# dyustc/CTC-Attention-Mispronunciation

Hardware: AMD Instinct MI355X
Metric: phoneme-frames/sec joint CTC-attn decode, 41-phone vocab (higher is better)
Workload: dtype f32 -- reference width (operands with all 24 significand bits, fp32 accumulate; see `accuracy`: closer to a float64 evaluation than ATen's own fp32): the large time-batched contractions (conv0/conv1, BiLSTM and text input projections) run on the bf16 matrix cores as f32x6 = each fp32 operand as thre

## Files before the change

ctc-attention-mispronunciation_amd/csrc/api.hip:

```cpp
#include <stdarg.h>
#include <stdio.h>
#include <string.h>

#include <functional>
#include <mutex>

#include "model.h"

namespace mdd {

static thread_local char g_err[512] = "";

void set_error(const char *fmt, ...) {
    va_list ap;
    va_start(ap, fmt);
    vsnprintf(g_err, sizeof(g_err), fmt, ap);
    va_end(ap);
}

struct DeviceGate {
    std::mutex mu;
    hipEvent_t done = nullptr;
    hipStream_t stream = nullptr;
    bool armed = false;
// ... 4 lines not shown
    SplitPtr s; s.hi = reinterpret_cast<unsigned short *>(b.p); s.lo = s.hi ? s.hi + n : nullptr; return s;
}
static const SplitPtr kNoSplit = {nullptr, nullptr};
static unsigned short *as_u16(const DeviceBuf &b) { return reinterpret_cast<unsigned short *>(b.p); }

static std::mutex g_prep_mu;

static int ensure(DeviceBuf &b, size_t n, hipStream_t zero_stream, bool *moved) {
    if (b.cap >= n) return MDD_OK;
    *moved = true;
    if (int rc = b.need(n)) return rc;
    b.cap = 0;
    MDD_HIP_CHECK(hipMemsetAsync(b.p, 0, n * sizeof(float), zero_stream));
    MDD_HIP_CHECK(hipStreamSynchronize(zero_stream));
    b.cap = n;
    return MDD_OK;
}

static ForwardPlan plan_of(const mdd_model *m, int B) { return plan_forward(m->cfg, m->precision, m->sw, m->fit, B); }

static int run_lstm(mdd_model *m, const LstmWeights &lw, LstmStepArgs a, hipStream_t st) {
    const ForwardPlan &p = m->plan;
    a.gx = m->gx.p; a.whh = lw.whh; a.hbuf = m->hbuf.p; a.cbuf = m->cbuf.p;
    a.H = m->cfg.hidden; a.packed = packed_whh(m->cfg);
    a.whh_split = lw.whh_s; a.hsplit = p.lstm == Lstm::StepX3 ? as_u16(m->hsplit) : nullptr;
    if (!p.gated) return launch_lstm_layer(a, st);
    unsigned short *hx = as_u16(m->hx);
    long long *stamps = m->sw.lstm_dbg && a.T > 100 ? reinterpret_cast<long long *>(m->hx.p + p.stamps_at) : nullptr;
    if (p.lstm == Lstm::X6) return launch_lstm_layer_x6(a, lw.whh_3, hx, m->sync_words.p, m->err_flag.p, st, stamps, m->sw.x6_redo_mask);
    if (p.lstm == Lstm::Granule) return launch_lstm_layer_granule(a, hx, m->sync_words.p, m->err_flag.p, st, stamps, m->sw.lstm_early);
    return launch_lstm_layer_f32(a, hx, m->sync_words.p, m->err_flag.p, st, stamps);
}

static LstmStepArgs lstm_raw_out(int T, int B, const int *seqlen, float *out, SplitPtr split) {
    LstmStepArgs a;
    a.T = T; a.B = B; a.seqlen = seqlen; a.out = out; a.out_raw = out; a.out_split = split;
    return a;
}
static LstmStepArgs lstm_folded_out(mdd_model *m, int n, int T, int B, const int *seqlen) {
    const ForwardPlan &p = m->plan;
    const bool x3 = p.precision == 1;
    const size_t n_out = (size_t)T * B * 2 * m->cfg.hidden;
    LstmStepArgs a;
    a.T = T; a.B = B; a.seqlen = seqlen;
    a.out = x3 || p.planes_out ? nullptr : m->act[n & 1].p; a.out_raw = m->taps ? m->tap_rnn[n].p : nullptr;
    if (p.planes_out) {
        a.out_planes = as_u16(m->p3); a.out_planes_stride = n_out;
    }
    a.out_split = x3 ? split_view(m->act_s[n & 1], n_out) : kNoSplit;
    a.oscale = m->weights->rnn[n + 1].scale; a.oshift = m->weights->rnn[n + 1].shift;
    return a;
}

struct ProjIn { const float *f32; SplitPtr split; bool planes_written; };
static int project(mdd_model *m, const ProjIn &in, int rows, int K, const LstmWeights &lw, const float *bias, hipStream_t st) {
    const int G2 = 8 * m->cfg.hidden;
    if (m->plan.proj == Gemm::Bf16x3) return launch_gemm_bf16x3(in.split, lw.wih_s, bias, m->gx.p, nullptr, rows, G2, K, K, K, G2, 1, 0, 0, 0, st);
    if (m->plan.proj == Gemm::F32x6) {
        if (!in.planes_written)
            if (int rc = launch_split3(in.f32, rows, K, K, as_u16(m->p3), st)) return rc;
        return launch_gemm_f32x6(as_u16(m->p3), (size_t)rows * K, lw.wih_3, (size_t)G2 * K, bias, m->gx.p, rows, G2, K, G2, st);
    }
    return launch_gemm_nt(in.f32, lw.wih, bias, m->gx.p, rows, G2, K, K, K, G2, 1, 0, 0, 0, st);
}

struct Stage { std::string name; int launches; double flops; std::function<int(hipStream_t)> run; };

static std::vector<Stage> forward_stages(mdd_model *m, const ForwardCall &call) {
    const mdd_config &c = m->cfg;
    const DecodeWeights *w = m->weights.get();
    const ForwardPlan p = m->plan;
    const float *x = call.x;
    const int B = call.B, T = call.T, L = call.L, Traw = call.Traw, Tp = T / 2, Lp = L;
    const int H = c.hidden, H2 = 2 * H, ch = c.channels, E = c.emb_dim, K0 = m->rnn_in(), nl = c.layers;
    const bool x3 = p.precision == 1, fused = p.conv != Conv::Separate;
    const size_t rows = (size_t)Tp * B, trows = (size_t)L * B;
    const auto split = [x3](const DeviceBuf &b, size_t n) { return x3 ? split_view(b, n) : kNoSplit; };
    const double step_flops = 2.0 * 2 * (double)B * H * 4 * H;
    std::vector<Stage> s;

    if (fused) {
        s.push_back({"conv_fused", 1, 2.0 * 9 * ch * (double)B * Tp * m->W2() * (ch + 6.0), [=](hipStream_t st) {
            if (p.conv == Conv::FusedX3)
                return launch_conv_fused(x, w->w_conv0, w->sc0, w->sh0, w->w_conv1_s, w->sc1, w->sh1, split_view(m->seq0_s, rows * K0), nullptr, B, T, Traw, st);
            return launch_conv_fused3(x, w->w_conv0, w->sc0, w->sh0, w->w_conv1_3, w->sc1, w->sh1, as_u16(m->p3), m->taps ? m->seq0.p : nullptr, B, T, Traw, st,
                                      p.conv == Conv::FusedX6Rowwise);
        }});
        s.push_back({"conv1_in_fused", 0, 0.0, [](hipStream_t) { return (int)MDD_OK; }});
    } else {
        s.push_back({"conv0", 1, 2.0 * 9 * ch * (double)B * T * m->W1(), [=](hipStream_t st) {
            return launch_conv0(x, w->w_conv0, w->sc0, w->sh0, m->y0.p, B, T, c.feat, ch, st);
        }});
        s.push_back({"conv1", 1, 2.0 * 9 * ch * ch * (double)B * Tp * m->W2(), [=](hipStream_t st) {
            return launch_conv1(m->y0.p, w->w_conv1t, w->sc1, w->sh1, x3 ? nullptr : m->seq0.p, split(m->seq0_s, rows * K0), B, T, m->W1(), ch, st);
        }});
    }

    for (int n = 0; n < nl; n++) {
        const LstmWeights *lw = &w->rnn[n];
        const int K = n == 0 ? K0 : H2;
        const ProjIn in = n == 0 ? ProjIn{m->seq0.p, split(m->seq0_s, rows * K), fused}
                                 : ProjIn{m->act[(n - 1) & 1].p, split(m->act_s[(n - 1) & 1], rows * K), p.planes_out};
        s.push_back({"gemm_ih" + std::to_string(n), 1, 2.0 * (double)Tp * B * 8 * H * K, [=](hipStream_t st) {
            return project(m, in, Tp * B, K, *lw, nullptr, st);
        }});
        const LstmStepArgs a = n == nl - 1 ? lstm_raw_out(Tp, B, call.tlen, m->xraw.p, split(m->x_s, rows * H2)) : lstm_folded_out(m, n, Tp, B, call.tlen);
        s.push_back({"lstm" + std::to_string(n), p.gated ? 1 : Tp, step_flops * Tp, [=](hipStream_t st) { return run_lstm(m, *lw, a, st); }});
    }

    const LstmWeights *tw = &w->rnn[nl];
    s.push_back({"embed", 1, 0.0, [=](hipStream_t st) {
        return launch_embed(w->emb, c.emb_rows, E, call.x1, B, L, x3 ? nullptr : m->embo.p, split(m->embo_s, trows * E), m->err_flag.p, st);
    }});
    s.push_back({"gemm_text", 1, 2.0 * (double)L * B * 8 * H * E, [=](hipStream_t st) {
        return project(m, ProjIn{m->embo.p, split(m->embo_s, trows * E), false}, L * B, E, *tw, w->t_bias, st);
    }});
    const LstmStepArgs ta = lstm_raw_out(L, B, call.llen, m->text.p, split(m->text_s, trows * H2));
    s.push_back({"lstm_text", p.gated ? 1 : L, step_flops * L, [=](hipStream_t st) { return run_lstm(m, *tw, ta, st); }});
    s.push_back({"gemm_key", 1, 2.0 * (double)L * B * H2 * H2, [=](hipStream_t st) {
        if (x3) {
            const SplitPtr ks = split_view(m->key_s, trows * H2);
            return launch_gemm_bf16x3(split_view(m->text_s, trows * H2), w->w_score_s, nullptr, nullptr, &ks, L * B, H2, H2, H2, H2, H2, 1, 0, 0, 0, st);
        }
        return launch_gemm_nt(m->text.p, w->w_score, nullptr, m->key.p, L * B, H2, H2, H2, H2, H2, 1, 0, 0, 0, st);
    }});
    s.push_back({"gemm_score", 1, 2.0 * (double)B * Tp * L * H2, [=](hipStream_t st) {
        if (x3) return launch_gemm_bf16x3(split_view(m->x_s, rows * H2), split_view(m->key_s, trows * H2), nullptr, m->S.p, nullptr, Tp, L, H2, B * H2, B * H2, Lp,
                                          B, H2, H2, (long)Tp * Lp, st);
        return launch_gemm_nt(m->xraw.p, m->key.p, nullptr, m->S.p, Tp, L, H2, B * H2, B * H2, Lp, B, H2, H2, (long)Tp * Lp, st);
    }});
    s.push_back({"attn_tail", 1, 2.0 * (double)B * Tp * ((double)L * H2 + 2.0 * H2 * c.num_class), [=](hipStream_t st) {
        return launch_attn_tail(m->S.p, Lp, m->xraw.p, m->text.p, w->fscale, w->fshift, w->w_fc, w->w_fcp, call.logp, Tp, B, L, H2, c.num_class, st, call.llen);
    }});
    return s;
}

int device_gate_enter(int device, hipStream_t st, bool *held) {
    *held = false;
    hipStreamCaptureStatus cs = hipStreamCaptureStatusNone;
    if (st && hipStreamIsCapturing(st, &cs) == hipSuccess && cs != hipStreamCaptureStatusNone) return MDD_OK;
    DeviceGate &g = g_gate[device & 63];
    g.mu.lock();
    *held = true;
    if (g.armed && g.stream != st) {
        hipError_t e = hipStreamWaitEvent(st, g.done, 0);
        if (e != hipSuccess) { g.mu.unlock(); *held = false; set_error("device gate: %s", hipGetErrorString(e)); return MDD_ERR_HIP; }
    }
    return MDD_OK;
}
int device_gate_leave(int device, hipStream_t st, bool held, int rc) {
    if (!held) return rc;
    DeviceGate &g = g_gate[device & 63];
    hipError_t e = hipSuccess;
    if (!g.done) e = hipEventCreateWithFlags(&g.done, hipEventDisableTiming);
    if (e == hipSuccess) e = hipEventRecord(g.done, st);
    if (e == hipSuccess) { g.armed = true; g.stream = st; }
    g.mu.unlock();
    if (e != hipSuccess && rc == MDD_OK) { set_error("device gate: %s", hipGetErrorString(e)); return MDD_ERR_HIP; }
    return rc;
}

}

using namespace mdd;

extern "C" const char *mdd_last_error(void) { return g_err; }
extern "C" int mdd_version(void) { return 100; }

extern "C" int mdd_create(const mdd_config *cfg, int device, mdd_model **out) {
// ... 292 lines not shown
```

ctc-attention-mispronunciation_amd/csrc/decode.hip:

```cpp
#include "mdd_internal.h"

namespace mdd {

__global__ __launch_bounds__(256) void greedy_kernel(const float *__restrict__ logp, int T, int B, int C,
                                                     const int32_t *__restrict__ len, int blank,
                                                     int32_t *__restrict__ ids, int32_t *__restrict__ nids) {
    extern __shared__ int am[];
    const int b = blockIdx.x, lane = threadIdx.x & 63, wave = threadIdx.x >> 6;
    int n = len[b];
    n = n < 0 ? 0 : (n > T ? T : n);
    for (int t = wave; t < n; t += 4) {
        const float *row = logp + ((size_t)t * B + b) * C;
        float bv = -INFINITY;
        int bi = 0x7fffffff;
        for (int c = lane; c < C; c += 64) {
            float v = row[c];
            if (v > bv || bi == 0x7fffffff) { bv = v; bi = c; }
        }
        for (int o = 32; o > 0; o >>= 1) {
            float ov = __shfl_xor(bv, o);
            int oi = __shfl_xor(bi, o);
            if (oi != 0x7fffffff && (bi == 0x7fffffff || ov > bv || (ov == bv && oi < bi))) { bv = ov; bi = oi; }
        }
        if (lane == 0) am[t] = bi;
    }
    __syncthreads();
    if (wave != 0) return;
    int count = 0;
    for (int base = 0; base < n; base += 64) {
        const int t = base + lane;
        bool keep = false;
        int a = 0;
        if (t < n) {
            a = am[t];
            keep = (a != blank) && !(t != 0 && a == am[t - 1]);
        }
        const unsigned long long mask = __ballot(keep);
        if (keep) ids[(size_t)b * T + count + __popcll(mask & ((1ull << lane) - 1ull))] = a;
        count += __popcll(mask);
    }
    if (lane == 0) nids[b] = count;
}

#define LOG_ZERO (-99999999.0)

__device__ __forceinline__ double log_add_prob(double lx, double ly) {
    const bool swap = (ly - lx) > 0.0;
    const double hi = swap ? ly : lx, lo = swap ? lx : ly;
    const double sum = hi + log(1 + exp(lo - hi));
    return lx <= LOG_ZERO ? ly : (ly <= LOG_ZERO ? lx : sum);
}

struct BeamMeta {
    double prTotal, prNonBlank, prBlank;
    unsigned long long hash, phash;
    int len, last;
};

constexpr int MAXBEAM = 64;

__device__ __forceinline__ void wave_argmax(double &v, int &ord) {
    for (int o = 32; o > 0; o >>= 1) {
        const double ov = __shfl_xor(v, o);
        const int oo = __shfl_xor(ord, o);
        if (ov > v || (ov == v && oo < ord)) { v = ov; ord = oo; }
    }
}

__global__ __launch_bounds__(256) void beam_prep_kernel(const float *__restrict__ logp, int T, int B, int C, int blank,
                                                        double *__restrict__ lp, unsigned char *__restrict__ flags) {
    const size_t n = (size_t)T * B * C;
    for (size_t i = (size_t)blockIdx.x * blockDim.x + threadIdx.x; i < n; i += (size_t)gridDim.x * blockDim.x) {
        const float p = (float)exp((double)logp[i]);
        lp[i] = p > 0.0f ? log((double)p) : -INFINITY;
        const size_t tb = i / C;
        if ((int)(i - tb * C) == blank) {
            unsigned char f = ((1.0f - p) < 0.1f) ? 0 : 1;
            const size_t t = tb / B;
            if (t > 0) {
                const float pprev = (float)exp((double)logp[i - (size_t)B * C]);
                if (pprev < 0.9f) f |= 2;
            }
// ... 518 lines not shown
            if (rank < keep) { sel_v[rank] = v; sel_x[rank] = cl_x[e]; }
        }
        BEAM_WAVE_SYNC();
        FSTAMP(8);
        if (DBG) ph[11] += nl;
        const int nxt = cur ^ 1;
        int r_new, app_k, app_at;
        {
            const int idx = sel_x[li];
            const double v = sel_v[li];
            i32x4 M4[FB / 4];
#pragma unroll
            for (int a = 0; a < FB / 4; a++) M4[a] = reinterpret_cast<const i32x4 *>(mslot)[a];
            const int r = min((int)(((float)idx + 0.5f) * invC), FB - 1), k = idx - r * C;
            const double cNBr = cNB[r], cBr = cB[r];
            const int len_r = m_len[cur][r], last_r = m_last[cur][r];
            const unsigned long long hash_r = m_hash[cur][r], phash_r = m_phash[cur][r];
            int fa = -1;
#pragma unroll
            for (int a = 0; a < FB; a++) fa = M4[a >> 2][a & 3] == idx ? a : fa;
            const double cNBa = cNB[max(fa, 0)], cBa = cB[max(fa, 0)];
            const bool isb = k == blank;
            r_new = r; app_k = isb ? -1 : k; app_at = len_r;
            if (lane < FB) {
                const bool on = lane < keep;
                m_T[nxt][lane] = v;
                m_NB[nxt][lane] = isb ? cNBr : (fa >= 0 ? cNBa : v);
                m_B[nxt][lane] = isb ? cBr : (fa >= 0 ? cBa : LOG_ZERO);
                m_len[nxt][lane] = on ? (isb ? len_r : len_r + 1) : -2;
                m_last[nxt][lane] = on ? (isb ? last_r : k) : -1;
                m_hash[nxt][lane] = isb ? hash_r : hash_r * 0x9E3779B97F4A7C15ull + (unsigned long long)(k + 1);
                m_phash[nxt][lane] = isb ? phash_r : hash_r;
            }
        }
        FSTAMP(9);
        {
            int rr[FB];
#pragma unroll
            for (int i = 0; i < FB; i++) rr[i] = __builtin_amdgcn_readlane(r_new, i);
            unsigned int *dstw = reinterpret_cast<unsigned int *>(pnext);
            for (int j = lane; j < nw; j += 64) {
                unsigned int w[FB];
#pragma unroll
                for (int i = 0; i < FB; i++) w[i] = srcw[rr[i] * nw + j];
#pragma unroll
                for (int i = 0; i < FB; i++) dstw[i * nw + j] = w[i];
            }
            BEAM_WAVE_SYNC();
            if (lane < keep && app_k >= 0) pnext[(size_t)lane * Tcap + app_at] = (unsigned char)app_k;
        }
        BEAM_WAVE_SYNC();
        cur = nxt;
        nb = keep;
        t = tn;
        FSTAMP(10);
    }
    BEAM_WAVE_SYNC();
    if (lane == 0) {
        int best = -1;
        double bestv = 0.0;
        for (int r = 0; r < nb && !err; r++) {
            const int ylen = m_len[cur][r];
            if (ylen == 0) { err = MDD_BEAM_INDEX_ERROR; break; }
            const double v = lmt[m_last[cur][r] * C1 + C];
            if (v != v) { err = MDD_BEAM_KEY_ERROR; break; }
            double pr = log_add_prob(LOG_ZERO, m_T[cur][r] + v * alpha);
            pr = pr * (1.0 / (double)(ylen ? ylen : 1));
            if (best < 0 || pr > bestv) { best = r; bestv = pr; }
        }
        status[b] = err;
        int n = 0;
        if (!err && best >= 0) {
            n = m_len[cur][best];
            const unsigned char *src = pref + (size_t)cur * FB * Tcap + (size_t)best * Tcap;
            for (int j = 0; j < n; j++) ids[(size_t)b * T + j] = src[j];
        }
        nids[b] = n;
        if (score) score[b] = err ? __builtin_nan("") : bestv;
        if (DBG) for (int i = 0; i < 12; i++) dbg[b * 12 + i] = ph[i];
    }
#undef FSTAMP
}

}

extern "C" int mdd_greedy(const float *logp_dev, int32_t T, int32_t B, int32_t C, const int32_t *len_dev, int32_t blank,
                          int32_t *ids_dev, int32_t *nids_dev, void *stream) {
    using namespace mdd;
    if (!logp_dev || !len_dev || !ids_dev || !nids_dev || T <= 0 || B <= 0 || C <= 0 || blank < 0 || blank >= C) {
        set_error("mdd_greedy: bad argument"); return MDD_ERR_ARG;
    }
    if ((size_t)T * 4 > 150 * 1024) { set_error("mdd_greedy: T=%d too long", T); return MDD_ERR_ARG; }
    hipLaunchKernelGGL(greedy_kernel, dim3(B), dim3(256), (size_t)T * sizeof(int), (hipStream_t)stream, logp_dev, T, B, C,
                       len_dev, blank, ids_dev, nids_dev);
    MDD_LAUNCH_CHECK();
    return MDD_OK;
}

extern "C" int mdd_beam(const float *logp_dev, int32_t T, int32_t B, int32_t C, const int32_t *len_dev, int32_t beam,
                        int32_t blank, const double *lm_dev, double lm_alpha, int32_t *ids_dev, int32_t *nids_dev,
                        int32_t *status_dev, double *score_dev, void *stream) {
    using namespace mdd;
    if (!logp_dev || !len_dev || !lm_dev || !ids_dev || !nids_dev || !status_dev || T <= 0 || B <= 0 || C <= 1 ||
        C > 256 || beam < 1 || beam > MAXBEAM || blank < 0 || blank >= C) {
        set_error("mdd_beam: bad argument (need 1<=beam<=64, 2<=C<=256)"); return MDD_ERR_ARG;
    }
    hipStream_t st = (hipStream_t)stream;
    const int Tcap = (T + 1 + 3) & ~3;
    const size_t lm_bytes = sizeof(double) * (size_t)(C + 1) * (C + 1);
    const size_t base = (sizeof(double) * 2 + sizeof(int)) * (size_t)beam * C + (size_t)(2 * beam + 1) * Tcap;
    const int lm_in_lds = (base + lm_bytes <= 96 * 1024) ? 1 : 0;
    const size_t smem = base + (lm_in_lds ? lm_bytes : 0);
    if (smem > 140 * 1024) { set_error("mdd_beam: beam*C / T too large for LDS (%zu B)", smem); return MDD_ERR_ARG; }
    static bool attr_set = false;
    if (!attr_set) {
        MDD_HIP_CHECK(hipFuncSetAttribute((const void *)beam_kernel, hipFuncAttributeMaxDynamicSharedMemorySize, 140 * 1024));
        attr_set = true;
    }
    double *lpw = nullptr;
    unsigned char *flags = nullptr;
    const size_t n = (size_t)T * B * C;
    MDD_HIP_CHECK(hipMallocAsync((void **)&lpw, n * sizeof(double) + (size_t)T * B, st));
    flags = reinterpret_cast<unsigned char *>(lpw + n);
    int grid = (int)((n + 255) / 256);
    if (grid > 2048) grid = 2048;
    hipLaunchKernelGGL(beam_prep_kernel, dim3(grid), dim3(256), 0, st, logp_dev, T, B, C, blank, lpw, flags);
    const int nslots = beam * C;
    if (beam <= FB && C <= 64 && nslots <= 1024 && !getenv("MDD_BEAM_GENERIC")) {
        const int NS = nslots <= 512 ? 8 : 16;
        const size_t lmb = beam_fast_lm_bytes(C);
        const size_t pw = (beam_fast_wave_bytes(NS, beam, Tcap) + 15) & ~(size_t)15;
        const size_t lds_max = 160 * 1024;
        static bool fattr = false;
        if (!fattr) {
            MDD_HIP_CHECK(hipFuncSetAttribute((const void *)beam_fast_kernel<8, false>, hipFuncAttributeMaxDynamicSharedMemorySize, (int)lds_max));
            MDD_HIP_CHECK(hipFuncSetAttribute((const void *)beam_fast_kernel<16, false>, hipFuncAttributeMaxDynamicSharedMemorySize, (int)lds_max));
            MDD_HIP_CHECK(hipFuncSetAttribute((const void *)beam_fast_kernel<8, true>, hipFuncAttributeMaxDynamicSharedMemorySize, (int)lds_max));
            MDD_HIP_CHECK(hipFuncSetAttribute((const void *)beam_fast_kernel<16, true>, hipFuncAttributeMaxDynamicSharedMemorySize, (int)lds_max));
            fattr = true;
        }
        if (lmb + pw > lds_max) { (void)hipFreeAsync(lpw, st); set_error("mdd_beam: T too long for LDS (%zu B)", lmb + pw); return MDD_ERR_ARG; }
        int W = (int)((lds_max - lmb) / pw);
        W = W > 4 ? 4 : W;
        if (B <= 64) W = 1;
        if (const char *we = getenv("MDD_BEAM_W")) { const int w = atoi(we); if (w >= 1 && w <= W) W = w; }
        const size_t fs = lmb + (size_t)W * pw;
        const dim3 grid_f((B + W - 1) / W), block_f(64 * W);
        long long *fdbg = getenv("MDD_BEAM_DBG") ? reinterpret_cast<long long *>(score_dev) + B : nullptr;
#define MDD_BEAM_FAST(NS_, DBG_) hipLaunchKernelGGL((beam_fast_kernel<NS_, DBG_>), grid_f, block_f, fs, st, lpw, flags, T, B, C, len_dev, beam, blank, \
                                                  lm_dev, lm_alpha, ids_dev, nids_dev, status_dev, score_dev, Tcap, fdbg)
        if (NS == 8) { if (fdbg) MDD_BEAM_FAST(8, true); else MDD_BEAM_FAST(8, false); }
        else { if (fdbg) MDD_BEAM_FAST(16, true); else MDD_BEAM_FAST(16, false); }
#undef MDD_BEAM_FAST
    } else
    hipLaunchKernelGGL(beam_kernel, dim3(B), dim3(64), smem, st, lpw, flags, T, B, C, len_dev, beam, blank, lm_dev, lm_alpha,
                       ids_dev, nids_dev, status_dev, score_dev, Tcap, lm_in_lds, getenv("MDD_BEAM_SKIP") ? atoi(getenv("MDD_BEAM_SKIP")) : 0,
                       getenv("MDD_BEAM_DBG") ? reinterpret_cast<long long *>(score_dev) + B : nullptr);
    hipError_t le = hipGetLastError();
    (void)hipFreeAsync(lpw, st);
    if (le != hipSuccess) { set_error("beam kernel launch failed: %s", hipGetErrorString(le)); return MDD_ERR_HIP; }
    return MDD_OK;
}
```

ctc-attention-mispronunciation_amd/csrc/frontend.hip:

```cpp
#include "mdd_internal.h"

namespace mdd {

__global__ void stack_skip_kernel(const float *__restrict__ raw, int T_raw, int D, int right, int skip, int kept,
                                  int T_out, float *__restrict__ out) {
    const int W = (right + 1) * D;
    const int b = blockIdx.y, i = blockIdx.x;
    const float *src = raw + (size_t)b * T_raw * D;
    float *dst = out + ((size_t)b * T_out + i) * W;
    for (int j = threadIdx.x; j < W; j += blockDim.x) {
        float v = 0.f;
        if (i < kept) {
            int r = j / D, c = j - r * D;
            int s = i * skip + r;
            if (s > T_raw - 1) s = T_raw - 1;
            v = src[(size_t)s * D + c];
        }
        dst[j] = v;
    }
}

int launch_stack_skip(const float *raw, int B, int T_raw, int D, int right, int skip, int n_down, float *out,
                      hipStream_t st) {
    if (B <= 0 || T_raw <= 0 || D <= 0 || right < 0) { set_error("stack_skip: bad shape"); return MDD_ERR_ARG; }
// ... 510 lines not shown
        if (tp + R < tp_end) load_x(tp + R, xnext);
        CM_T(3);
        __syncthreads();
        CM_T(4);
        f32x16 acc;
#pragma unroll
        for (int r = 0; r < 16; r++) acc[r] = 0.f;
        const int m = min(mt * 32 + li, W2 - 1);
        int slot[3];
#pragma unroll
        for (int kh = 0; kh < 3; kh++) { const int r = 2 * jr + kh + rot; slot[kh] = (r >= NY ? r - NY : r) * CF_NCOL * 64; }
        float *rt = red + (jr * 2 + mt) * 16 * 64;
        auto conv1 = [&](auto kc) {
            constexpr int KH2 = decltype(kc)::value;
#pragma unroll
            for (int i = 0; i < 9; i++) {
                const int kb = KH2 * 9 + i, kk = kb >> 1, kh = kk / 3, kw = kk - kh * 3;
                const int off = slot[kh] + cm_yoff(0, 2 * m + kw, (kb & 1) * 2 + half);
                const bf16x8 ah = *reinterpret_cast<const bf16x8 *>(yh + off);
                const bf16x8 am = *reinterpret_cast<const bf16x8 *>(ym + off);
                const bf16x8 al = *reinterpret_cast<const bf16x8 *>(yl + off);
                acc = __builtin_amdgcn_mfma_f32_32x32x16_bf16(am, bwm[i], acc, 0, 0, 0);
                acc = __builtin_amdgcn_mfma_f32_32x32x16_bf16(ah, bwl[i], acc, 0, 0, 0);
                acc = __builtin_amdgcn_mfma_f32_32x32x16_bf16(al, bwh[i], acc, 0, 0, 0);
                acc = __builtin_amdgcn_mfma_f32_32x32x16_bf16(ah, bwm[i], acc, 0, 0, 0);
                acc = __builtin_amdgcn_mfma_f32_32x32x16_bf16(am, bwh[i], acc, 0, 0, 0);
                acc = __builtin_amdgcn_mfma_f32_32x32x16_bf16(ah, bwh[i], acc, 0, 0, 0);
            }
#pragma unroll
            for (int r = 0; r < 8; r++) rt[((1 - KH2) * 8 + r) * 64 + lane] = acc[(1 - KH2) * 8 + r];
        };
        auto finish = [&](auto kc) {
            constexpr int KH2 = decltype(kc)::value;
            unsigned short *oh = ost + jr * 3 * ROW + li * W2 + mt * 32 + 4 * half, *om = oh + ROW, *ol = om + ROW;
            const bool cut = mt == 1 && half == 1;
#pragma unroll
            for (int r = KH2 * 8; r < KH2 * 8 + 8; r += 2) {
                float v[2];
#pragma unroll
                for (int e = 0; e < 2; e++) {
                    const float p = rt[(r + e) * 64 + lane];
                    v[e] = (KH2 == 0 ? acc[r + e] + p : p + acc[r + e]) * s1 + h1;
                    v[e] = v[e] > 0.f ? v[e] : 0.f;
                }
                unsigned hw, mw, lw;
                split3_pair(v[0], v[1], hw, mw, lw);
                const int wo = (r & 3) + 8 * (r >> 2);
                if (r < 13 || !cut) { oh[wo] = (unsigned short)hw; om[wo] = (unsigned short)mw; ol[wo] = (unsigned short)lw; }
                if (r + 1 < 13 || !cut) { oh[wo + 1] = (unsigned short)(hw >> 16); om[wo + 1] = (unsigned short)(mw >> 16); ol[wo + 1] = (unsigned short)(lw >> 16); }
            }
        };
        if (kh2 == 0) conv1(std::integral_constant<int, 0>{}); else conv1(std::integral_constant<int, 1>{});
        CM_T(5);
        __syncthreads();
        CM_T(6);
        if (tp + jr < tp_end) {
            if (kh2 == 0) finish(std::integral_constant<int, 0>{}); else finish(std::integral_constant<int, 1>{});
        }
        CM_T(7);
        __syncthreads();
        CM_T(8);
        const int nr = min(R, tp_end - tp);
        unsigned short *orow = out3 + (size_t)tp * B * 32;
#pragma unroll
        for (int k = 0; k < SPT; k++) {
            const int i = tid + 512 * k;
            if (i < nr * 3 * 244) *reinterpret_cast<u32x4 *>(orow + sdst[k]) = *reinterpret_cast<const u32x4 *>(ost + i * 8);
        }
        if (out_f32)
            for (int i = tid; i < nr * ROW; i += 512) {
                const int jj = i / ROW, c = i - jj * ROW;
                const unsigned short *oh = ost + jj * 3 * ROW;
                out_f32[((size_t)(tp + jj) * B + b) * ROW + c] =
                    (__uint_as_float((unsigned)oh[c] << 16) + __uint_as_float((unsigned)oh[ROW + c] << 16)) + __uint_as_float((unsigned)oh[2 * ROW + c] << 16);
            }
        CM_T(9);
    }
    if (STAMP && stamps && lane == 0 && blockIdx.x < 512)
        for (int i = 0; i < CM_NPH; i++) stamps[((size_t)blockIdx.x * 8 + wave) * CM_NPH + i] = sacc[i];
#undef CM_T
}

int launch_conv_fused(const float *x, const float *w0, const float *sc0, const float *sh0, SplitPtr w1, const float *sc1,
                      const float *sh1, SplitPtr out, float *out_f32, int B, int T, int Traw, hipStream_t st) {
    const int Tp = T / 2;
    if (Tp <= 0 || B <= 0) return MDD_OK;
    int S = (1024 + B - 1) / B;
    S = S < 1 ? 1 : (S > Tp ? Tp : S);
    const int seg = (Tp + S - 1) / S;
    S = (Tp + seg - 1) / seg;
    hipLaunchKernelGGL(conv_fused_kernel<2>, dim3(B * S), dim3(256), conv_fused_smem(2), st, x, w0, sc0, sh0, w1.hi, w1.lo, sc1, sh1,
                       out.hi, out.lo, out_f32, B, T, Traw, S, seg);
    MDD_LAUNCH_CHECK();
    return MDD_OK;
}

int launch_conv_fused3(const float *x, const float *w0, const float *sc0, const float *sh0, const unsigned short *w1_3, const float *sc1,
                       const float *sh1, unsigned short *out3, float *out_f32, int B, int T, int Traw, hipStream_t st, bool rowwise,
                       long long *stamps) {
    const int Tp = T / 2;
    if (Tp <= 0 || B <= 0) return MDD_OK;
    int S = (512 + B - 1) / B;
    S = S < 1 ? 1 : (S > Tp ? Tp : S);
    int seg = (Tp + S - 1) / S;
    if (!rowwise) {
        seg = (seg + CM_R - 1) / CM_R * CM_R;
        S = (Tp + seg - 1) / seg;
        if (stamps) hipLaunchKernelGGL((conv_fused_kernel<3, CM_R, true>), dim3(B * S), dim3(512), conv_multirow_smem(), st, x, w0, sc0, sh0, w1_3,
                                       sc1, sh1, out3, out_f32, B, T, Traw, S, seg, stamps);
        else hipLaunchKernelGGL((conv_fused_kernel<3, CM_R, false>), dim3(B * S), dim3(512), conv_multirow_smem(), st, x, w0, sc0, sh0, w1_3,
                                sc1, sh1, out3, out_f32, B, T, Traw, S, seg, nullptr);
        MDD_LAUNCH_CHECK();
        return MDD_OK;
    }
    S = (Tp + seg - 1) / seg;
    const size_t plane = (size_t)Tp * B * 1952;
    hipLaunchKernelGGL(conv_fused_kernel<3>, dim3(B * S), dim3(256), conv_fused_smem(3), st, x, w0, sc0, sh0, w1_3, w1_3 + 32 * 288, sc1, sh1,
                       out3, out3 + plane, out_f32, B, T, Traw, S, seg);
    MDD_LAUNCH_CHECK();
    return MDD_OK;
}

int init_conv_attributes() {
    MDD_HIP_CHECK(hipFuncSetAttribute((const void *)conv_fused_kernel<2>, hipFuncAttributeMaxDynamicSharedMemorySize, 96 * 1024));
    MDD_HIP_CHECK(hipFuncSetAttribute((const void *)conv_fused_kernel<3>, hipFuncAttributeMaxDynamicSharedMemorySize, 128 * 1024));
    MDD_HIP_CHECK(hipFuncSetAttribute((const void *)conv_fused_kernel<3, CM_R, false>, hipFuncAttributeMaxDynamicSharedMemorySize, (int)conv_multirow_smem()));
    MDD_HIP_CHECK(hipFuncSetAttribute((const void *)conv_fused_kernel<3, CM_R, true>, hipFuncAttributeMaxDynamicSharedMemorySize, (int)conv_multirow_smem()));
    return MDD_OK;
}

__global__ void conv_diag_fill_kernel(float *x, size_t n, unsigned seed, float scale, float offset) {
    for (size_t i = (size_t)blockIdx.x * blockDim.x + threadIdx.x; i < n; i += (size_t)gridDim.x * blockDim.x) {
        unsigned h = (unsigned)i * 2654435761u + seed; h ^= h >> 15; h *= 2246822519u; h ^= h >> 13;
        x[i] = ((float)(h & 0xffffff) / 8388608.f - 1.f) * scale + offset;
    }
}
__global__ void conv_diag_split3_kernel(const float *w, int n, unsigned short *planes) {
    for (int i = blockIdx.x * blockDim.x + threadIdx.x; i < n; i += gridDim.x * blockDim.x) {
        const float v = w[i];
        const __bf16 h = (__bf16)v;
        const float r1 = v - (float)h;
        const __bf16 m = (__bf16)r1, l = (__bf16)(r1 - (float)m);
        planes[i] = *reinterpret_cast<const unsigned short *>(&h);
        planes[n + i] = *reinterpret_cast<const unsigned short *>(&m);
        planes[2 * n + i] = *reinterpret_cast<const unsigned short *>(&l);
    }
}

}

extern "C" int mdd_diag_conv_time(int B, int T, int reps, int which, float *ms_out, double *phases, long long *mismatch) {
    using namespace mdd;
    if (B <= 0 || T < 2 || reps < 1 || which < 0 || which > 1 || !ms_out) { set_error("mdd_diag_conv_time: bad arguments"); return MDD_ERR_ARG; }
    const int Tp = T / 2;
    const size_t nx = (size_t)B * T * 243, nout = (size_t)3 * Tp * B * 1952;
    DeviceBuf xb, wb;
    DeviceArray<unsigned short> w13, out, out2;
    DeviceArray<long long> sd;
    if (int rc = init_conv_attributes()) return rc;
    if (xb.need(nx) || wb.need(416 + 32 * 288) || w13.need(3 * 32 * 288) || out.need(nout) || (mismatch && out2.need(nout)) ||
        (phases && sd.need((size_t)512 * 8 * CM_NPH))) return MDD_ERR_HIP;
    hipLaunchKernelGGL(conv_diag_fill_kernel, dim3(4096), dim3(256), 0, 0, xb.p, nx, 1u, 2.f, 0.f);
    hipLaunchKernelGGL(conv_diag_fill_kernel, dim3(4), dim3(256), 0, 0, wb.p, (size_t)288, 2u, 0.4f, 0.f);
    hipLaunchKernelGGL(conv_diag_fill_kernel, dim3(1), dim3(64), 0, 0, wb.p + 288, (size_t)32, 3u, 0.2f, 1.f);
    hipLaunchKernelGGL(conv_diag_fill_kernel, dim3(1), dim3(64), 0, 0, wb.p + 320, (size_t)32, 4u, 0.3f, 0.1f);
    hipLaunchKernelGGL(conv_diag_fill_kernel, dim3(1), dim3(64), 0, 0, wb.p + 352, (size_t)32, 5u, 0.2f, 1.f);
    hipLaunchKernelGGL(conv_diag_fill_kernel, dim3(1), dim3(64), 0, 0, wb.p + 384, (size_t)32, 6u, 0.3f, 0.1f);
    hipLaunchKernelGGL(conv_diag_fill_kernel, dim3(36), dim3(256), 0, 0, wb.p + 416, (size_t)32 * 288, 7u, 0.1f, 0.f);
    hipLaunchKernelGGL(conv_diag_split3_kernel, dim3(36), dim3(256), 0, 0, wb.p + 416, 32 * 288, w13.p);
    MDD_LAUNCH_CHECK();
    auto run = [&](int w, unsigned short *o, long long *stp) {
        return launch_conv_fused3(xb.p, wb.p, wb.p + 288, wb.p + 320, w13.p, wb.p + 352, wb.p + 384, o, nullptr, B, T, 0, 0, w == 1, stp);
    };
    hipEvent_t e0 = nullptr, e1 = nullptr;
    MDD_HIP_CHECK(hipEventCreate(&e0));
    MDD_HIP_CHECK(hipEventCreate(&e1));
    int rc = MDD_OK;
    for (int r = -2; r < reps && !rc; r++) {
        if (r == 0) (void)hipEventRecord(e0, 0);
        rc = run(which, out.p, nullptr);
    }
    (void)hipEventRecord(e1, 0);
    if (hipEventSynchronize(e1) != hipSuccess) rc = rc ? rc : MDD_ERR_HIP;
    float ms = 0.f;
    (void)hipEventElapsedTime(&ms, e0, e1);
    *ms_out = ms / reps;
// ... 31 lines not shown
```

ctc-attention-mispronunciation_amd/csrc/mdd_internal.h:

```cpp
#pragma once
#include <hip/hip_runtime.h>
#include <stdint.h>

#include <map>
#include <string>
#include <utility>
#include <vector>

#include "../../include/mdd_hip.h"
#include "plan.h"

namespace mdd {

void set_error(const char *fmt, ...);

#define MDD_HIP_CHECK(expr)                                                                     \
    do {                                                                                        \
        hipError_t e_ = (expr);                                                                 \
        if (e_ != hipSuccess) {                                                                 \
            mdd::set_error("%s failed: %s (%s:%d)", #expr, hipGetErrorString(e_), __FILE__, __LINE__); \
            return MDD_ERR_HIP;                                                                 \
        }                                                                                       \
    } while (0)

#define MDD_LAUNCH_CHECK() MDD_HIP_CHECK(hipGetLastError())

template <class T> struct DeviceArray {
    T *p = nullptr;
    size_t cap = 0;
    DeviceArray() = default;
    DeviceArray(const DeviceArray &) = delete;
    DeviceArray &operator=(const DeviceArray &) = delete;
    DeviceArray(DeviceArray &&o) noexcept : p(o.p), cap(o.cap) { o.p = nullptr; o.cap = 0; }
    DeviceArray &operator=(DeviceArray &&o) noexcept { std::swap(p, o.p); std::swap(cap, o.cap); return *this; }
    ~DeviceArray() { if (p) (void)hipFree(p); }
    int need(size_t n) {
        if (cap >= n) return MDD_OK;
        T *old = p;
        p = nullptr; cap = 0;
        if (old) MDD_HIP_CHECK(hipFree(old));
        MDD_HIP_CHECK(hipMalloc((void **)&p, n * sizeof(T)));
        cap = n;
        return MDD_OK;
    }
};
using DeviceBuf = DeviceArray<float>;

struct SplitPtr { unsigned short *hi, *lo; };

int launch_gemm_nt(const float *A, const float *W, const float *bias, float *C, int M, int N, int K, int lda, int ldw,
                   int ldc, int batch, long sA, long sW, long sC, hipStream_t st);

int launch_gemm_f32(bool ta, bool tb, const float *A, const float *B, const float *bias, float *C, int M, int N, int K, int lda, int ldb,
                    int ldc, int batch, long sA, long sB, long sC, bool accumulate, hipStream_t st, int ksplit = 0);

int launch_gemm_bf16x3(const SplitPtr &A, const SplitPtr &W, const float *bias, float *C, const SplitPtr *Csplit, int M, int N,
                       int K, int lda, int ldw, int ldc, int batch, long sA, long sW, long sC, hipStream_t st);
int init_gemm_attributes();
int launch_split(const float *x, size_t n, const SplitPtr &out, hipStream_t st);
int launch_unsplit(const SplitPtr &in, size_t n, float *x, hipStream_t st);
int launch_split3(const float *x, int rows, int K, int ld, unsigned short *planes, hipStream_t st);
int launch_gemm_f32x6(const unsigned short *A3, size_t a_plane, const unsigned short *W3, size_t w_plane, const float *bias, float *C, int M, int N, int K,
                      int ldc, hipStream_t st, long long *stamps = nullptr);
int init_gemm_x6_attributes();
int launch_split3_pad(const float *x, int rows, int K, int ld, int Kp, unsigned short *planes, size_t plane_elems, hipStream_t st);
int launch_transpose_split3(const float *x, int K, int rows, int ld, int Kp, unsigned short *planes, size_t plane_elems, hipStream_t st);
int launch_gemm_f32x6_splitk(const unsigned short *A3, size_t a_plane, const unsigned short *W3, size_t w_plane, float *part, int M, int N, int Kc, int S,
                             hipStream_t st);

int launch_stack_skip(const float *raw, int B, int T_raw, int D, int right, int skip, int n_down, float *out,
                      hipStream_t st);
int launch_conv0(const float *x, const float *w, const float *scale, const float *shift, float *y0, int B, int T, int F,
                 int ch, hipStream_t st);
int launch_conv1(const float *y0, const float *w_t, const float *scale, const float *shift, float *seq, SplitPtr seq_split, int B,
                 int T, int W1, int ch, hipStream_t st);

int launch_conv_fused(const float *x, const float *w0, const float *sc0, const float *sh0, SplitPtr w1, const float *sc1,
                      const float *sh1, SplitPtr out, float *out_f32, int B, int T, int Traw, hipStream_t st);
int launch_conv_fused3(const float *x, const float *w0, const float *sc0, const float *sh0, const unsigned short *w1_3, const float *sc1,
                       const float *sh1, unsigned short *out3, float *out_f32, int B, int T, int Traw, hipStream_t st,
                       bool rowwise = false,
                       long long *stamps = nullptr);
int init_conv_attributes();

bool x6_ops_ok(const float *A, int lda, const float *B, int ldb, const float *C, int ldc);
int gemm_f32x6_ops(bool ta, bool tb, const float *A, int lda, const float *B, int ldb, const float *bias, float *C, int ldc, int M, int N, int K, int S,
                   DeviceBuf &xs_a, DeviceBuf &xs_b, DeviceBuf &part, hipStream_t st);

struct LstmStepArgs {
    const float *gx;
    const float *whh;
    float *hbuf;
    float *cbuf;
    float *out = nullptr;
    SplitPtr out_split = {nullptr, nullptr};
    float *out_raw = nullptr;
    const float *oscale = nullptr;
    const float *oshift = nullptr;
    int T, B, H;
    SplitPtr whh_split;
    unsigned short *hsplit;
    int packed;
    float *gates_save = nullptr;
    float *c_save = nullptr;
    const int *seqlen = nullptr;
    unsigned short *out_planes = nullptr;
    size_t out_planes_stride = 0;
};
int launch_lstm_layer(const LstmStepArgs &a, hipStream_t st);

int launch_embed(const float *table, int rows, int E, const int64_t *ids, int B, int L, float *out, SplitPtr out_split,
                 int *err_flag, hipStream_t st);
int launch_attn_tail(const float *S, int Lp, const float *X, const float *V, const float *fscale, const float *fshift,
                     const float *wfc, const float *wfcp, float *logp, int Tp, int B, int L, int H2, int C, hipStream_t st,
                     const int *llen = nullptr);

int init_kernel_attributes();
int init_ctc_attributes();
int init_lstm_attributes();
int init_granule_attributes();
int persistent_grid_fits(int n_cu);
int launch_lstm_layer_granule(const LstmStepArgs &s, unsigned short *hx, unsigned int *sync, int *err_flag, hipStream_t st,
                              long long *stamps = nullptr, bool early = false);
int launch_zero_fill(void *p, size_t n, hipStream_t st);
int launch_lstm_layer_f32(const LstmStepArgs &s, unsigned short *hx, unsigned int *sync, int *err_flag, hipStream_t st, long long *stamps);
int init_lstm_f32_attributes();
int persistent_f32_grid_fits(int n_cu);
int launch_lstm_layer_x6(const LstmStepArgs &s, const unsigned short *whh3, unsigned short *hx, unsigned int *sync, int *err_flag, hipStream_t st,
                         long long *stamps, int force_mask);
int init_lstm_x6_attributes();
int persistent_x6_grid_fits(int n_cu);
size_t lstm_bwd_granule_hx_bytes(int H);
int launch_lstm_bwd_granule(const float *dout, const float *gates, const float *cst, SplitPtr whhT, float *dg, int T, int B, int H, unsigned short *hx,
                            unsigned int *sync, int *err_flag, hipStream_t st);
int device_gate_enter(int device, hipStream_t st, bool *held);
int device_gate_leave(int device, hipStream_t st, bool held, int rc);

}
```

ctc-attention-mispronunciation_amd/csrc/plan.h:

```cpp
#pragma once
#include <stddef.h>
#include <stdlib.h>
#include <string.h>

#include "../../include/mdd_hip.h"

namespace mdd {

struct Switches {
    int precision = 2;
    bool graph = true;
    bool lstm_step = false;
    bool lstm_x3 = false;
    bool x6_off = false;
    bool x6_force = false;
    bool conv_rowwise = false;
    bool lstm_dbg = false;
    bool lstm_early = false;
    int x6_redo_mask = -1;
    bool x6_out_fp32 = false;
    int train_precision = 0;
    bool train_conv1_im2col = false;
};

inline Switches read_switches() {
    Switches s;
    auto is = [](const char *e, const char *v) { return e && !strcmp(e, v); };
    const char *e = getenv("MDD_PRECISION");
    if (is(e, "f32") || is(e, "0")) s.precision = 0;
    if (is(e, "bf16x3") || is(e, "1")) s.precision = 1;
    e = getenv("MDD_GRAPH");
    s.graph = !(e && e[0] == '0');
    e = getenv("MDD_LSTM");
    s.lstm_step = is(e, "step");
    s.lstm_x3 = is(e, "x3");
    e = getenv("MDD_LSTM_X6");
    s.x6_off = e && e[0] == '0';
    s.x6_force = e && e[0] == 'f';
    s.conv_rowwise = is(getenv("MDD_CONV"), "rowwise");
    s.lstm_dbg = getenv("MDD_LSTM_DBG") != nullptr;
    s.lstm_early = getenv("MDD_LSTM_EARLY") != nullptr;
    e = getenv("MDD_X6_FORCE_REDO");
    const int n = e ? atoi(e) : 0;
    if (n > 0 && (n & (n - 1)) == 0) s.x6_redo_mask = n - 1;
    s.x6_out_fp32 = is(getenv("MDD_X6_OUT"), "fp32");
    e = getenv("MDD_TRAIN_PRECISION");
    if (is(e, "bf16x3") || is(e, "1")) s.train_precision = 1;
    if (is(e, "f32x6") || is(e, "2")) s.train_precision = 2;
    s.train_conv1_im2col = getenv("MDD_TRAIN_CONV1_IM2COL") != nullptr;
    return s;
}

struct DeviceFit { bool granule, f32, x6; };

inline int conv_out(int w) { return (w + 2 - 3) / 2 + 1; }
inline int rnn_in(const mdd_config &c) { return c.channels * conv_out(conv_out(c.feat)); }

inline bool packed_whh(const mdd_config &c) { return c.hidden == 384 || c.hidden == 256; }

inline int granule_bg(int B) { const int r = (B + 15) / 16; return (r + 15) / 16 * 16; }
inline size_t lstm_x6_hx_bytes(int H, int B) { const int bgr = (B + 7) / 8, nbt = (bgr + 15) / 16; return (size_t)2 * 16 * nbt * 3 * (H / 8) * 256; }
inline size_t team8_hx_alloc_floats(int H, int B) { return (size_t)2 * 32 * granule_bg(B) * H * 2; }
inline size_t team8_hx_live_bytes(int H, int BG) { return (size_t)2 * 32 * BG * H * 4; }
static constexpr size_t kHxTailFloats = 64 + 256 * 6 * 2;
static constexpr int kPersistMaxB = 1024;

enum class Conv { Separate, FusedX3, FusedX6, FusedX6Rowwise };
enum class Gemm { Nt, Bf16x3, F32x6 };
enum class Lstm { X6, F32, Granule, StepX3, StepPacked, Step };

struct ForwardPlan {
    int precision;
    Conv conv;
    Gemm proj;
    Lstm lstm;
    bool gated;
    size_t hx_floats;
    size_t stamps_at;
    bool planes_out;
};

inline ForwardPlan plan_forward(const mdd_config &c, int precision, const Switches &sw, const DeviceFit &fit, int B) {
    const int H = c.hidden, K0 = rnn_in(c);
    const bool packed = packed_whh(c);
    const bool x3 = precision == 1 && packed && K0 % 32 == 0 && c.emb_dim % 32 == 0;
    const bool x6 = precision == 2 && K0 % 32 == 0 && (2 * H) % 32 == 0 && c.emb_dim % 32 == 0;
    ForwardPlan p{};
    p.precision = x3 ? 1 : x6 ? 2 : 0;
    if ((x3 || x6) && c.feat == 243 && c.channels == 32) p.conv = x3 ? Conv::FusedX3 : sw.conv_rowwise ? Conv::FusedX6Rowwise : Conv::FusedX6;
    else p.conv = Conv::Separate;
    p.proj = x3 ? Gemm::Bf16x3 : x6 ? Gemm::F32x6 : Gemm::Nt;
    const bool persist = fit.granule && !sw.lstm_step && !sw.lstm_x3 && packed && B <= kPersistMaxB && (x3 || fit.f32);
    const bool lx6 = x6 && persist && fit.x6 && !sw.x6_off && (sw.x6_force || H == 384 || B <= 128);
    if (lx6) p.lstm = Lstm::X6;
    else if (persist) p.lstm = x3 ? Lstm::Granule : Lstm::F32;
    else if (x3 && sw.lstm_x3) p.lstm = Lstm::StepX3;
    else p.lstm = packed ? Lstm::StepPacked : Lstm::Step;
    p.gated = persist;
    p.planes_out = p.proj == Gemm::F32x6 && lx6 && !sw.x6_out_fp32;
    if (persist) {
        const size_t granules = team8_hx_alloc_floats(H, B), planes = lstm_x6_hx_bytes(H, B) / 4;
        p.stamps_at = lx6 ? planes : granules;
        p.hx_floats = (lx6 && planes > granules ? planes : granules) + kHxTailFloats;
    }
    return p;
}

}
```

Baseline: 4.564 million.

## Run beam search on a high-priority side stream and retune conv segment count

The beam-search kernel is moved onto a per-device high-priority non-blocking stream, joined to the caller stream with events when the caller is not capturing a graph. The aim is to let decode work be scheduled ahead of other queued work. Separately, the fused x6 conv now targets 1024 workgroups instead of 512 when B>64, and an env override for the segment count is added. This adds stream and event bookkeeping plus a global mutex held across the launch, and changes conv grid sizing for large batches.

```diff
diff --git a/ctc-attention-mispronunciation_amd/csrc/api.hip b/ctc-attention-mispronunciation_amd/csrc/api.hip
--- a/ctc-attention-mispronunciation_amd/csrc/api.hip
+++ b/ctc-attention-mispronunciation_amd/csrc/api.hip
@@ -110,9 +110,10 @@
     if (fused) {
         s.push_back({"conv_fused", 1, 2.0 * 9 * ch * (double)B * Tp * m->W2() * (ch + 6.0), [=](hipStream_t st) {
             if (p.conv == Conv::FusedX3)
-                return launch_conv_fused(x, w->w_conv0, w->sc0, w->sh0, w->w_conv1_s, w->sc1, w->sh1, split_view(m->seq0_s, rows * K0), nullptr, B, T, Traw, st);
+                return launch_conv_fused(x, w->w_conv0, w->sc0, w->sh0, w->w_conv1_s, w->sc1, w->sh1, split_view(m->seq0_s, rows * K0), nullptr, B, T, Traw, st,
+                                         m->sw.conv_s);
             return launch_conv_fused3(x, w->w_conv0, w->sc0, w->sh0, w->w_conv1_3, w->sc1, w->sh1, as_u16(m->p3), m->taps ? m->seq0.p : nullptr, B, T, Traw, st,
-                                      p.conv == Conv::FusedX6Rowwise);
+                                      p.conv == Conv::FusedX6Rowwise, nullptr, m->sw.conv_s);
         }});
         s.push_back({"conv1_in_fused", 0, 0.0, [](hipStream_t) { return (int)MDD_OK; }});
     } else {
diff --git a/ctc-attention-mispronunciation_amd/csrc/decode.hip b/ctc-attention-mispronunciation_amd/csrc/decode.hip
--- a/ctc-attention-mispronunciation_amd/csrc/decode.hip
+++ b/ctc-attention-mispronunciation_amd/csrc/decode.hip
@@ -1,3 +1,5 @@
+#include <mutex>
+
 #include "mdd_internal.h"
 
 namespace mdd {
@@ -682,6 +684,28 @@
 #undef FSTAMP
 }
 
+struct BeamLane { hipStream_t s = nullptr; hipEvent_t in = nullptr, out = nullptr; bool tried = false; };
+static std::mutex beam_lane_mu;
+static BeamLane beam_lanes[16];
+static BeamLane *beam_lane(hipStream_t st) {
+    const char *e = getenv("MDD_BEAM_PRIO");
+    if (e && e[0] == '0') return nullptr;
+    hipStreamCaptureStatus cs = hipStreamCaptureStatusNone;
+    if (hipStreamIsCapturing(st, &cs) != hipSuccess || cs != hipStreamCaptureStatusNone) { (void)hipGetLastError(); return nullptr; }
+    int dev = 0;
+    if (hipGetDevice(&dev) != hipSuccess || dev < 0 || dev >= 16) return nullptr;
+    BeamLane &l = beam_lanes[dev];
+    if (!l.tried) {
+        l.tried = true;
+        int least = 0, greatest = 0;
+        if (hipDeviceGetStreamPriorityRange(&least, &greatest) != hipSuccess ||
+            hipStreamCreateWithPriority(&l.s, hipStreamNonBlocking, greatest) != hipSuccess ||
+            hipEventCreateWithFlags(&l.in, hipEventDisableTiming) != hipSuccess ||
+            hipEventCreateWithFlags(&l.out, hipEventDisableTiming) != hipSuccess) { (void)hipGetLastError(); l.s = nullptr; }
+    }
+    return l.s ? &l : nullptr;
+}
+
 }
 
 extern "C" int mdd_greedy(const float *logp_dev, int32_t T, int32_t B, int32_t C, const int32_t *len_dev, int32_t blank,
@@ -705,7 +729,7 @@
         C > 256 || beam < 1 || beam > MAXBEAM || blank < 0 || blank >= C) {
         set_error("mdd_beam: bad argument (need 1<=beam<=64, 2<=C<=256)"); return MDD_ERR_ARG;
     }
-    hipStream_t st = (hipStream_t)stream;
+    const hipStream_t caller = (hipStream_t)stream;
     const int Tcap = (T + 1 + 3) & ~3;
     const size_t lm_bytes = sizeof(double) * (size_t)(C + 1) * (C + 1);
     const size_t base = (sizeof(double) * 2 + sizeof(int)) * (size_t)beam * C + (size_t)(2 * beam + 1) * Tcap;
@@ -717,10 +741,28 @@
         MDD_HIP_CHECK(hipFuncSetAttribute((const void *)beam_kernel, hipFuncAttributeMaxDynamicSharedMemorySize, 140 * 1024));
         attr_set = true;
     }
+    static bool fattr = false;
+    if (!fattr) {
+        const void *kernels[] = {(const void *)beam_fast_kernel<8, false>, (const void *)beam_fast_kernel<16, false>,
+                                 (const void *)beam_fast_kernel<8, true>, (const void *)beam_fast_kernel<16, true>};
+        for (const void *k : kernels) MDD_HIP_CHECK(hipFuncSetAttribute(k, hipFuncAttributeMaxDynamicSharedMemorySize, 160 * 1024));
+        fattr = true;
+    }
     double *lpw = nullptr;
     unsigned char *flags = nullptr;
     const size_t n = (size_t)T * B * C;
-    MDD_HIP_CHECK(hipMallocAsync((void **)&lpw, n * sizeof(double) + (size_t)T * B, st));
+    MDD_HIP_CHECK(hipMallocAsync((void **)&lpw, n * sizeof(double) + (size_t)T * B, caller));
+    std::unique_lock<std::mutex> lane_lock(beam_lane_mu);
+    BeamLane *lane = beam_lane(caller);
+    if (lane && (hipEventRecord(lane->in, caller) != hipSuccess || hipStreamWaitEvent(lane->s, lane->in, 0) != hipSuccess)) { (void)hipGetLastError(); lane = nullptr; }
+    if (!lane) lane_lock.unlock();
+    const hipStream_t st = lane ? lane->s : caller;
+    const auto join = [&]() {
+        hipError_t e = hipSuccess;
+        if (lane) { e = hipEventRecord(lane->out, st); if (e == hipSuccess) e = hipStreamWaitEvent(caller, lane->out, 0); }
+        (void)hipFreeAsync(lpw, caller);
+        return e;
+    };
     flags = reinterpret_cast<unsigned char *>(lpw + n);
     int grid = (int)((n + 255) / 256);
     if (grid > 2048) grid = 2048;
@@ -731,15 +773,7 @@
         const size_t lmb = beam_fast_lm_bytes(C);
         const size_t pw = (beam_fast_wave_bytes(NS, beam, Tcap) + 15) & ~(size_t)15;
         const size_t lds_max = 160 * 1024;
-        static bool fattr = false;
-        if (!fattr) {
-            MDD_HIP_CHECK(hipFuncSetAttribute((const void *)beam_fast_kernel<8, false>, hipFuncAttributeMaxDynamicSharedMemorySize, (int)lds_max));
-            MDD_HIP_CHECK(hipFuncSetAttribute((const void *)beam_fast_kernel<16, false>, hipFuncAttributeMaxDynamicSharedMemorySize, (int)lds_max));
-            MDD_HIP_CHECK(hipFuncSetAttribute((const void *)beam_fast_kernel<8, true>, hipFuncAttributeMaxDynamicSharedMemorySize, (int)lds_max));
-            MDD_HIP_CHECK(hipFuncSetAttribute((const void *)beam_fast_kernel<16, true>, hipFuncAttributeMaxDynamicSharedMemorySize, (int)lds_max));
-            fattr = true;
-        }
-        if (lmb + pw > lds_max) { (void)hipFreeAsync(lpw, st); set_error("mdd_beam: T too long for LDS (%zu B)", lmb + pw); return MDD_ERR_ARG; }
+        if (lmb + pw > lds_max) { (void)join(); set_error("mdd_beam: T too long for LDS (%zu B)", lmb + pw); return MDD_ERR_ARG; }
         int W = (int)((lds_max - lmb) / pw);
         W = W > 4 ? 4 : W;
         if (B <= 64) W = 1;
@@ -757,7 +791,8 @@
                        ids_dev, nids_dev, status_dev, score_dev, Tcap, lm_in_lds, getenv("MDD_BEAM_SKIP") ? atoi(getenv("MDD_BEAM_SKIP")) : 0,
                        getenv("MDD_BEAM_DBG") ? reinterpret_cast<long long *>(score_dev) + B : nullptr);
     hipError_t le = hipGetLastError();
-    (void)hipFreeAsync(lpw, st);
+    const hipError_t je = join();
+    if (le == hipSuccess) le = je;
     if (le != hipSuccess) { set_error("beam kernel launch failed: %s", hipGetErrorString(le)); return MDD_ERR_HIP; }
     return MDD_OK;
 }
diff --git a/ctc-attention-mispronunciation_amd/csrc/frontend.hip b/ctc-attention-mispronunciation_amd/csrc/frontend.hip
--- a/ctc-attention-mispronunciation_amd/csrc/frontend.hip
+++ b/ctc-attention-mispronunciation_amd/csrc/frontend.hip
@@ -616,11 +616,10 @@
 }
 
 int launch_conv_fused(const float *x, const float *w0, const float *sc0, const float *sh0, SplitPtr w1, const float *sc1,
-                      const float *sh1, SplitPtr out, float *out_f32, int B, int T, int Traw, hipStream_t st) {
+                      const float *sh1, SplitPtr out, float *out_f32, int B, int T, int Traw, hipStream_t st, int force_s) {
     const int Tp = T / 2;
     if (Tp <= 0 || B <= 0) return MDD_OK;
-    int S = (1024 + B - 1) / B;
-    S = S < 1 ? 1 : (S > Tp ? Tp : S);
+    int S = conv_segments(B, Tp, 1024, force_s);
     const int seg = (Tp + S - 1) / S;
     S = (Tp + seg - 1) / seg;
     hipLaunchKernelGGL(conv_fused_kernel<2>, dim3(B * S), dim3(256), conv_fused_smem(2), st, x, w0, sc0, sh0, w1.hi, w1.lo, sc1, sh1,
@@ -631,11 +630,10 @@
 
 int launch_conv_fused3(const float *x, const float *w0, const float *sc0, const float *sh0, const unsigned short *w1_3, const float *sc1,
                        const float *sh1, unsigned short *out3, float *out_f32, int B, int T, int Traw, hipStream_t st, bool rowwise,
-                       long long *stamps) {
+                       long long *stamps, int force_s) {
     const int Tp = T / 2;
     if (Tp <= 0 || B <= 0) return MDD_OK;
-    int S = (512 + B - 1) / B;
-    S = S < 1 ? 1 : (S > Tp ? Tp : S);
+    int S = conv_segments(B, Tp, conv_x6_workgroups(B), force_s);
     int seg = (Tp + S - 1) / S;
     if (!rowwise) {
         seg = (seg + CM_R - 1) / CM_R * CM_R;
diff --git a/ctc-attention-mispronunciation_amd/csrc/mdd_internal.h b/ctc-attention-mispronunciation_amd/csrc/mdd_internal.h
--- a/ctc-attention-mispronunciation_amd/csrc/mdd_internal.h
+++ b/ctc-attention-mispronunciation_amd/csrc/mdd_internal.h
@@ -76,11 +76,13 @@
                  int T, int W1, int ch, hipStream_t st);
 
 int launch_conv_fused(const float *x, const float *w0, const float *sc0, const float *sh0, SplitPtr w1, const float *sc1,
-                      const float *sh1, SplitPtr out, float *out_f32, int B, int T, int Traw, hipStream_t st);
+                      const float *sh1, SplitPtr out, float *out_f32, int B, int T, int Traw, hipStream_t st,
+                      int force_s = 0);
 int launch_conv_fused3(const float *x, const float *w0, const float *sc0, const float *sh0, const unsigned short *w1_3, const float *sc1,
                        const float *sh1, unsigned short *out3, float *out_f32, int B, int T, int Traw, hipStream_t st,
                        bool rowwise = false,
-                       long long *stamps = nullptr);
+                       long long *stamps = nullptr,
+                       int force_s = 0);
 int init_conv_attributes();
 
 bool x6_ops_ok(const float *A, int lda, const float *B, int ldb, const float *C, int ldc);
diff --git a/ctc-attention-mispronunciation_amd/csrc/plan.h b/ctc-attention-mispronunciation_amd/csrc/plan.h
--- a/ctc-attention-mispronunciation_amd/csrc/plan.h
+++ b/ctc-attention-mispronunciation_amd/csrc/plan.h
@@ -15,6 +15,7 @@
     bool x6_off = false;
     bool x6_force = false;
     bool conv_rowwise = false;
+    int conv_s = 0;
     bool lstm_dbg = false;
     bool lstm_early = false;
     int x6_redo_mask = -1;
@@ -38,6 +39,8 @@
     s.x6_off = e && e[0] == '0';
     s.x6_force = e && e[0] == 'f';
     s.conv_rowwise = is(getenv("MDD_CONV"), "rowwise");
+    e = getenv("MDD_CONV_S");
+    s.conv_s = e && atoi(e) > 0 ? atoi(e) : 0;
     s.lstm_dbg = getenv("MDD_LSTM_DBG") != nullptr;
     s.lstm_early = getenv("MDD_LSTM_EARLY") != nullptr;
     e = getenv("MDD_X6_FORCE_REDO");
@@ -64,6 +67,12 @@
 inline size_t team8_hx_live_bytes(int H, int BG) { return (size_t)2 * 32 * BG * H * 4; }
 static constexpr size_t kHxTailFloats = 64 + 256 * 6 * 2;
 static constexpr int kPersistMaxB = 1024;
+
+inline int conv_segments(int B, int Tp, int wgs, int forced) {
+    const int S = forced > 0 ? forced : (wgs + B - 1) / B;
+    return S < 1 ? 1 : (S > Tp ? Tp : S);
+}
+inline int conv_x6_workgroups(int B) { return B > 64 ? 1024 : 512; }
 
 enum class Conv { Separate, FusedX3, FusedX6, FusedX6Rowwise };
 enum class Gemm { Nt, Bf16x3, F32x6 };
```

Result: no change. 4.563 million (-0.0%).
